# mathwrx/Decouple-and-Couple_Learning_in_Multi-Modal_Brain_Tumor_Segmentation

Measured on AMD Instinct MI355X. Metric: training volumes/sec (4x128^3), higher is better.
Workload: dtype bf16x3 forward (split-bf16 MFMA operands hi.hi+hi.lo+lo.hi: logits within 1e-3 of the fp32 reference) / bf16 data-gradient / bf16 weight-gradient MFMA operands; f32 accumulate, f32 storage, f32 master weights; 1 GPU; configs[1]: 1xMI355X, batch 2 per GPU, 4-modality 128^3 synthetic BraTS patches; fwd + softmax_dice + 4 sub-region/edge losses + bwd + Adam(amsgrad); random-init weights, dropout on; global_batch=2, parallelism=dp1, precision=bf16x3, dgrad_precision=bf16, wgrad_precision=bf16, mode=plan

## Files before the change

### decouple-and-couple_learning_in_multi-modal_brain_tumor_segmentation_amd/csrc/conv_wsp.hip

```cpp
#include "conv_args.h"
#include <cstdlib>
#include <type_traits>

#define WSP_ID 6
#define WSP_IH 6
#define WSP_IW 18
#define WSP_NVOX (WSP_ID * WSP_IH * WSP_IW)
#define WSP_SLOTS 11
#define WSP_NT 2
#define WSP_NBW 14

struct WspWork { int ngroups, slots, tiles, xcd_perm, stat_rows; };

__host__ __device__ constexpr int wsp_tap_bytes(int t) { return (((t / 9) * WSP_IH + (t / 3) % 3) * WSP_IW + t % 3) * 32; }

template <int T>
__global__ __launch_bounds__(512) void convwsp_kernel(const ConvArgsB a, const WspWork wk) {
  constexpr int NT = WSP_NT;
  constexpr int B_IMG = 14 * NT * 1024;
  constexpr int A_IMG = WSP_NVOX * 32;
  constexpr int A_BUF = 2 * A_IMG;
  extern __shared__ float4 lds4[];
  char* lds = reinterpret_cast<char*>(lds4);
  char* const Bh = lds;
// ... 164 lines not shown
      using I0 = std::integral_constant<int, 0>; using I1 = std::integral_constant<int, 1>;
#define WSP_IC(v) std::integral_constant<int, (v)>{}
#define WSP_STEP2(S0)                                                                                          \
      rd_lo(WSP_IC(S0)); rd_hi(WSP_IC((S0) + 1), I1{}); mm(I0{}); __builtin_amdgcn_sched_barrier(0);            \
      rd_lo(WSP_IC((S0) + 1)); if ((S0) + 2 < 14) rd_hi(WSP_IC((S0) + 2 < 14 ? (S0) + 2 : 13), I0{});           \
      mm(I1{}); __builtin_amdgcn_sched_barrier(0);
      rd_hi(I0{}, I0{});
      WSP_STEP2(0) WSP_STEP2(2) WSP_STEP2(4) WSP_STEP2(6) WSP_STEP2(8) WSP_STEP2(10) WSP_STEP2(12)
#undef WSP_STEP2
#undef WSP_IC
    };

    int i = 0;
    for (int t0 = 0; t0 < ntw; t0 += T) {
      const int nk = min(T, ntw - t0);
      for (int c = 0; c < nch; ++c) {
        auto item = [&](auto KK) {
          constexpr int k = decltype(KK)::value;
          if (k == 0 && i > 0) asm volatile("s_barrier" ::: "memory");
          asm volatile("s_barrier" ::: "memory");
          mfma_item(i & 1, KK);
          if (c == nch - 1) epilogue(t_begin + t0 + k, KK);
          ++i;
        };
        item(std::integral_constant<int, 0>{});
        if (T > 1 && nk > 1) item(std::integral_constant<int, (T > 1 ? 1 : 0)>{});
        if (T > 2 && nk > 2) item(std::integral_constant<int, (T > 2 ? 2 : 0)>{});
        if (T > 3 && nk > 3) item(std::integral_constant<int, (T > 3 ? 3 : 0)>{});
      }
    }
    if (a.stats && stats_n >= 0) flush_stats();
  } else {
    const int tg = tid - 256;
    const int ni = ntw * nch;
    struct Item { int tile, chunk; bool first; };
    auto item_of = [&](int it) {
      const int per_round = T * nch;
      const int rd = it / per_round, w = it - rd * per_round;
      const int nk = min(T, ntw - rd * T);
      const int c = w / nk, k = w - c * nk;
      Item o; o.tile = t_begin + rd * T + k; o.chunk = c; o.first = k == 0;
      return o;
    };

    u32x4 wpf[WSP_NBW];
    const uint4* wsrc = a.wpk + (int64_t)g.cls_wbase16[0] * 128;
    auto w_issue = [&](int chunk) {
      int tgo = tg;
      asm volatile("" : "+v"(tgo));
#pragma unroll
      for (int i = 0; i < WSP_NBW; ++i) {
        const int e = tgo + 256 * i;
        const int img = e / (14 * NT * 64), e2 = e - img * (14 * NT * 64);
        const int ln = e2 & 63, blk = e2 >> 6;
        const int j = blk % NT, s = blk / NT;
        const uint4* p = wsrc + ((int64_t)(chunk * 14 + s) * g.ntiles + nt0 + j) * 128 + ln * 2 + img;
        wpf[i] = *reinterpret_cast<const u32x4*>(p);
      }
    };
    auto w_write = [&]() {
      int wb = tg * 16;
      asm volatile("" : "+v"(wb));
#pragma unroll
      for (int i = 0; i < WSP_NBW; ++i) *reinterpret_cast<u32x4*>(Bh + wb + i * 4096) = wpf[i];
    };

    const int q = tg & 3;
    const int vox0 = tg >> 2;
    const int iw_0 = vox0 % WSP_IW, row_0 = vox0 / WSP_IW;
    const bool plain = a.in_scale == nullptr && a.in_slope == 1.f;
    f32x4 pf[WSP_SLOTS];
    f32x4 pf_sc, pf_sh;
    unsigned pf_inb = 0u;
    auto issue = [&](int it) {
      const Item itm = item_of(it);
      const int tile = itm.tile, chunk = itm.chunk;
      const int n = tile / tiles_per_n;
      int bx = tile - n * tiles_per_n;
      const int tw = bx % g.tiles_w; bx /= g.tiles_w;
      const int th = bx % g.tiles_h, td = bx / g.tiles_h;
      const int id0 = td * 4 - 1, ih0 = th * 4 - 1, iw0 = tw * 16 - 1;
      const char* xb = reinterpret_cast<const char*>(a.x + (int64_t)n * g.Di * g.Hi * g.Wi * g.x_ldc + chunk * 16);
      const unsigned ldc4 = (unsigned)g.x_ldc * 4u;
      unsigned inb = 0u;
      int iw = iw_0, row = row_0;
      asm volatile("" : "+v"(iw), "+v"(row));
#pragma unroll
      for (int i = 0; i < WSP_SLOTS; ++i) {
        const int idd = (row * 43) >> 8, ih = row - idd * WSP_IH;
        const int gd = id0 + idd, gh = ih0 + ih, gw = iw0 + iw;
        const bool ok = (row < WSP_ID * WSP_IH) & ((unsigned)gd < (unsigned)g.Di) & ((unsigned)gh < (unsigned)g.Hi) & ((unsigned)gw < (unsigned)g.Wi);
        iw += 10; row += 3;
        if (iw >= WSP_IW) { iw -= WSP_IW; ++row; }
        const unsigned lin = (unsigned)((gd * g.Hi + gh) * g.Wi + gw) * ldc4 + (unsigned)q * 16u;
        const unsigned boff = ok ? lin : (unsigned)q * 16u;
        pf[i] = *reinterpret_cast<const f32x4*>(xb + boff);
        inb |= ok ? (1u << i) : 0u;
      }
      pf_inb = inb;
      const float* scp = a.in_scale ? a.in_scale + (int64_t)n * g.Cin + chunk * 16 : a.x;
      const float* shp = a.in_scale ? a.in_shift + (int64_t)n * g.Cin + chunk * 16 : a.x;
      pf_sc = *reinterpret_cast<const f32x4*>(reinterpret_cast<const char*>(scp) + q * 16);
      pf_sh = *reinterpret_cast<const f32x4*>(reinterpret_cast<const char*>(shp) + q * 16);
    };
    auto convert = [&](int buf) {
      const float slope = a.in_slope;
      const bool has_norm = a.in_scale != nullptr;
      const f32x4 sc = has_norm ? pf_sc : (f32x4){1.f, 1.f, 1.f, 1.f}, sh = has_norm ? pf_sh : (f32x4){0.f, 0.f, 0.f, 0.f};
      const unsigned inb = pf_inb;
      int vbase = (tg >> 2) * 32 + q * 8;
      asm volatile("" : "+v"(vbase));
      char* ah = A0 + buf * A_BUF + vbase;
#pragma unroll
      for (int i = 0; i < WSP_SLOTS; ++i) {
        if (i == WSP_SLOTS - 1 && vox0 + 64 * i >= WSP_NVOX) continue;
        float v0 = pf[i][0], v1 = pf[i][1], v2 = pf[i][2], v3 = pf[i][3];
        if (!plain) {
          v0 = act01(fmaf(v0, sc[0], sh[0]), slope); v1 = act01(fmaf(v1, sc[1], sh[1]), slope);
          v2 = act01(fmaf(v2, sc[2], sh[2]), slope); v3 = act01(fmaf(v3, sc[3], sh[3]), slope);
        }
        uint2 h, l;
        split_bf16(v0, v1, h.x, l.x); split_bf16(v2, v3, h.y, l.y);
        const bool was = (inb >> i) & 1u;
        h.x = was ? h.x : 0u; h.y = was ? h.y : 0u; l.x = was ? l.x : 0u; l.y = was ? l.y : 0u;
        *reinterpret_cast<uint2*>(ah + i * (64 * 32)) = h;
        *reinterpret_cast<uint2*>(ah + A_IMG + i * (64 * 32)) = l;
      }
    };

    __builtin_amdgcn_s_setprio(1);
    if (ni > 0) {
      issue(0);
      w_issue(0);
      convert(0);
      w_write();
      if (ni > 1) issue(1);
    }
    for (int it = 0; it < ni; ++it) {
      if (it > 0 && item_of(it).first) {
        asm volatile("s_barrier" ::: "memory");
        w_write();
      }
      asm volatile("s_waitcnt lgkmcnt(0)\n\ts_barrier" ::: "memory");
      if (it + 1 < ni) {
        convert((it + 1) & 1);
        const Item nx = item_of(it + 1);
        if (nx.first) w_issue(nx.chunk);
        if (it + 2 < ni) issue(it + 2);
      }
    }
  }
}

namespace {
template <int T>
int launch_wsp(const ConvArgsB& a, const WspWork& wk, int grid, hipStream_t st) {
  const size_t lds = (size_t)2 * 14 * WSP_NT * 1024 + (size_t)2 * 2 * WSP_NVOX * 32;
  CWF_MAX_LDS_ONCE((&convwsp_kernel<T>));
  hipLaunchKernelGGL((convwsp_kernel<T>), dim3(grid), dim3(512), lds, st, a, wk);
  CWF_LAUNCH_CHECK();
  return 0;
}
}

static int g_wsp = 1;
extern "C" int cwf_debug_wsp(int v) { const int old = g_wsp; g_wsp = v; return old; }
static long long g_wsp_launches = 0;
extern "C" long long cwf_debug_wsp_launches() { return g_wsp_launches; }
static const int g_wsp_min_cin = 128, g_wsp_min_units = 128;

int cwf_try_conv_wsp(int op, int x3, int cfg_mt, int cfg_wm, ConvArgsB& a, hipStream_t st, int* rc) {
  const ConvGeom& g = a.g;
  if (!g_wsp || !x3 || cwf_ws_takes_x3()) return 0;
  if (op != CWF_CONV3_S1 || a.groups || a.out_scale || a.nb_x) return 0;
  if (g.Cin < 32 || (g.Cin & 15) || (g.Cout & 31)) return 0;
  if ((g.Do & 3) || (g.Ho & 3) || (g.Wo & 15)) return 0;
  if (g.x_ldc < g.Cin || (g.x_ldc & 3)) return 0;
  if ((int64_t)g.Di * g.Hi * g.Wi * g.x_ldc * 4 >= (1ll << 31)) return 0;
  if (a.stats && !(cfg_mt == 1 || (cfg_mt == 4 && cfg_wm == 4))) return 0;
  WspWork wk;
  wk.stat_rows = cfg_mt;
  wk.ngroups = g.Cout / 32;
  if (wk.ngroups > 32) return 0;
  const int64_t tiles = (int64_t)g.N * (g.Do / 4) * (g.Ho / 4) * (g.Wo / 16);
  if (g_wsp == 1 && (g.Cin < g_wsp_min_cin || tiles * wk.ngroups < g_wsp_min_units)) return 0;
  int e = cwf_build_geom(a.g, op, g.N, g.Di, g.Hi, g.Wi, g.Cin, g.x_ldc, g.Do, g.Ho, g.Wo, g.Cout, g.y_ldc, 16);
  if (e) { *rc = e; return 1; }
  wk.tiles = (int)tiles;
  const int per = (32 / wk.ngroups) * wk.ngroups;
  wk.slots = 8 * (per / wk.ngroups);
  wk.xcd_perm = 1;
  if (wk.slots > wk.tiles) { wk.slots = wk.tiles; wk.xcd_perm = 0; }
  const int grid = wk.slots * wk.ngroups;
  const int per_wg = (wk.tiles + wk.slots - 1) / wk.slots;
  *rc = per_wg > 2 ? launch_wsp<4>(a, wk, grid, st) : launch_wsp<2>(a, wk, grid, st);
  if (*rc == 0) ++g_wsp_launches;
  return 1;
}
```

### decouple-and-couple_learning_in_multi-modal_brain_tumor_segmentation_amd/cwf/_lib.py

```python
from __future__ import annotations

import ctypes as C
import os

_HERE = os.path.dirname(os.path.abspath(__file__))
LIB_PATH = os.path.join(_HERE, "libcwf_hip.so")

P = C.c_void_p
I = C.c_int
L = C.c_int64
F = C.c_float
U = C.c_uint32
U64 = C.c_uint64
D = C.c_double

SIGNATURES = {
    "cwf_version": [],
    "cwf_conv": [P, P],
    "cwf_conv_x16_ok": [I, I, I, I, I, I, I],
    "cwf_debug_wsd": [I],
    "cwf_debug_wsd_launches": [],
    "cwf_wgrad": [P, P, P],
    "cwf_gather_split_bf16": [P, I, L, P],
    "cwf_wgrad_nsplit": [I, I, I, I, I, I, I],
    "cwf_wgrad_partial_floats": [I, I, I, I, I, I, I],
    "cwf_wgrad_slab_floats": [I, I, I],
    "cwf_wgrad_reduce": [P, I, L, P, P, P, P],
    "cwf_gather_batched": [P, I, L, P],
    "cwf_in_finalize": [P, P, P, I, L, F, P],
    "cwf_in_stats": [P, I, P, I, L, I, P],
    "cwf_norm_act_add": [P, I, P, P, F, P, I, P, I, I, L, I, P],
    "cwf_in_bwd_stats": [P, I, P, I, P, P, F, P, I, L, I, P],
    "cwf_in_bwd_apply": [P, I, P, I, P, P, F, P, P, I, P, I, I, L, I, P],
    "cwf_in_bwd_apply_ex": [P, I, P, I, P, P, F, P, P, I, P, I, P, P, I, L, I, P],
    "cwf_norm_act_add_ex": [P, I, P, P, F, P, I, P, I, P, I, L, I, P],
    "cwf_to_bf16": [P, I, P, P, F, P, I, L, I, P],
    "cwf_gemm": [P, L, L, L, L, P, L, L, L, L, P, L, L, L, P, P, L, L, L, I, I, I, I, I, F, I, I, P],
    "cwf_layernorm_fwd": [P, P, P, P, P, P, I, I, F, P],
    "cwf_layernorm_bwd": [P, P, P, P, P, P, P, P, I, I, I, P],
    "cwf_softmax_rows": [P, L, I, I, P],
    "cwf_softmax_rows_bwd": [P, P, L, I, I, P],
    "cwf_gelu_bwd": [P, P, P, L, P],
    "cwf_colsum": [P, L, I, I, P, I, P],
    "cwf_window_to_tokens": [P, I, P, I, I, I, I, I, I, I, I, P],
    "cwf_tokens_to_window": [P, P, I, I, I, I, I, I, I, I, I, I, P],
    "cwf_token_scores": [P, P, L, P, I, I, I, P],
    "cwf_topk": [P, P, I, I, I, P],
    "cwf_gather_tokens": [P, P, P, L, P, F, P, I, I, I, I, P],
    "cwf_gather_tokens_bwd": [P, P, P, P, P, L, I, I, I, I, P],
    "cwf_scatter_rows": [P, P, P, L, L, P, L, P, I, I, I, I, P],
    "cwf_scatter_rows_bwd": [P, P, P, P, L, P, I, P, L, L, P, L, I, I, I, I, P],
    "cwf_upsample_softmax": [P, I, P, I, I, I, I, I, I, P],
    "cwf_upsample_softmax_bwd": [P, P, P, I, I, I, I, I, I, I, P, P],
    "cwf_channel_softmax": [P, I, P, L, I, P],
    "cwf_channel_softmax_bwd": [P, P, P, I, L, I, P],
    "cwf_dice_ce_sums": [P, P, U, P, I, L, I, P],
    "cwf_dice_ce_finalize": [P, P, P, I, L, I, P],
    "cwf_dice_ce_bwd": [P, P, U, P, P, P, I, L, I, P],
    "cwf_adam_amsgrad": [P, I, L, C.c_double, C.c_double, C.c_double, C.c_double, C.c_double, I, I, P, P],
    "cwf_adam_amsgrad_scaled": [P, I, L, C.c_double, C.c_double, C.c_double, C.c_double, C.c_double, I, I, P, F, P],
    "cwf_grad_add": [P, P, P, L, P],
    "cwf_grad_norm_clip": [P, L, F, F, P, P, P],
    "cwf_adam_amsgrad_ex": [P, I, L, C.c_double, C.c_double, C.c_double, C.c_double, C.c_double, I, I, P, F, P, P, F, P],
    "cwf_optim_step": [I, P, I, L, C.c_double, C.c_double, P, C.c_double, C.c_double, C.c_double, I, I, P, C.c_double, C.c_double, I, I,
                       F, P, P, F, P],
    "cwf_wgrad_reduce_batched": [P, I, P],
    "cwf_dropout_mask": [P, L, F, F, C.c_uint64, C.c_uint64, P],
    "cwf_mul": [P, P, P, L, P],
    "cwf_add": [P, P, P, L, P],
    "cwf_channel_scale": [P, I, P, P, I, I, L, I, P],
    "cwf_copy_strided": [P, I, P, I, L, I, P],
    "cwf_add3": [P, P, P, P, L, P],
    "cwf_bcast3": [P, P, L, P],
    "cwf_stats_channel_sum": [P, P, I, I, P],
    "cwf_gemm_ex": [P, P],
    "cwf_attn_fwd": [P, L, P, L, I, I, I, I, F, P, U64, F, P],
    "cwf_attn_bwd": [P, L, P, L, P, I, I, I, I, F, P, U64, F, P],
    "cwf_ln_pair_fwd": [P, P, I, P, P, P, P, P, P, P, I, I, F, P],
    "cwf_ln_pair_bwd": [P, P, P, P, P, I, P, P, P, P, P, P, P, P, P, I, I, I, P],
    "cwf_gelu_bwd_drop": [P, P, P, L, P, U64, F, P],
    "cwf_token_scores2": [P, P, L, P, L, P, P, I, I, I, P],
    "cwf_topk_inv": [P, P, P, P, P, P, I, I, I, P],
    "cwf_index_inv": [P, P, I, I, I, P],
    "cwf_gather_multi": [P, I, I, I, I, F, P, F, P],
    "cwf_scatter_inv": [P, P, P, L, L, P, L, P, P, I, I, I, P],
    "cwf_scatter_bwd": [P, P, P, P, P, P, L, L, P, L, P, L, P, L, L, P, L, I, I, I, I, P],
    "cwf_token_grad": [P, P, P, L, P, P, P, L, P, L, P, U64, U64, F, P, I, I, I, I, P],
    "cwf_head_grad": [P, P, P, P, L, P, P, I, I, P],
    "cwf_dice_ce_finalize_multi": [P, P, P, P, I, I, L, I, P],
    "cwf_head_loss_sums": [P, I, I, P, P, P, I, I, I, I, I, P],
    "cwf_head_loss_bwd": [P, I, I, P, P, P, P, P, I, P, I, I, I, I, I, P],
    "cwf_head_loss_bwd_ex": [P, I, I, P, P, P, P, P, I, I, P, I, I, I, I, I, P],
    "cwf_ln_pair_fwd_g": [P, P, I, P, I, P, P, P, I, I, F, P],
    "cwf_ln_pair_bwd_g": [P, P, P, P, P, I, P, I, P, P, P, I, I, I, P],
    "cwf_token_scores2_g": [P, P, P, I, I, P, P, I, I, I, P],
    "cwf_head_grad_g": [P, P, P, P, L, P, P, I, I, I, P],
    "cwf_window_to_tokens_g": [P, I, P, I, I, I, I, I, I, I, I, I, P],
    "cwf_tokens_to_window_g": [P, P, I, I, I, I, I, I, I, I, I, I, P],
    "cwf_cat3_channels": [P, P, P, P, L, I, P],
    "cwf_stitch_windows": [P, P, I, P],
    "cwf_argmax_dice": [P, L, L, L, P, P, P, I, L, P],
    "cwf_argmax_metrics": [P, L, L, L, P, P, P, I, L, P],
    "cwf_region_bits": [P, P, L, P],
    "cwf_hausdorff_workspace": [I, I, I, I, I],
    "cwf_hausdorff": [P, P, I, I, I, I, I, D, D, D, I, I, P, P, P, P, L, P],
    "cwf_surface_metrics_workspace": [I, I, I, I, I],
    "cwf_surface_metrics": [P, P, I, I, I, I, I, D, D, D, I, I, P, I, P, P, P, P, P, P, P, P, L, P],
    "cwf_signed_distance_workspace": [I, I, I, I, I],
    "cwf_signed_distance": [P, P, P, I, I, I, I, I, P, P],
    "cwf_boundary_sums": [P, P, P, P, I, I, L, I, P],
    "cwf_boundary_finalize": [P, P, P, P, I, I, L, P],
    "cwf_boundary_bwd": [P, P, P, P, P, I, I, L, I, P],
    "cwf_topk_ce_workspace": [I, L],
    "cwf_topk_ce": [P, P, U, L, P, P, P, I, L, I, P, P],
    "cwf_topk_ce_bwd": [P, P, U, P, P, P, I, L, I, P],
    "cwf_focal_workspace": [I, L, I],
    "cwf_focal_loss": [P, P, P, I, P, P, P, P, I, L, I, P, P],
    "cwf_focal_loss_bwd": [P, P, P, I, P, P, P, P, I, L, I, P],
    "cwf_lovasz_workspace": [I, L, I],
    "cwf_lovasz": [P, P, P, I, I, P, P, P, P, I, L, P, P],
    "cwf_lovasz_bwd": [P, P, I, P, P, P, I, L, P],
    "cwf_components_workspace": [I, I, I, I, I],
    "cwf_components": [P, I, I, I, I, I, I, P, P, P, P, P, L, P],
    "cwf_postprocess_labels": [P, P, P, P, P, I, I, I, I, I, I, I, I, I, I, I, I, P, P, P],
    "cwf_label_metrics": [P, P, P, L, P],
    "cwf_dilate_bits": [P, P, I, I, I, I, I, I, P, L, P],
    "cwf_lesionwise_workspace": [I, I, I, I, I],
    "cwf_lesionwise": [P, P, I, I, I, I, I, I, L, D, P, P, P, P, P, P, L, P],
    "cwf_lesionwise_ex_workspace": [I, I, I, I, I],
    "cwf_lesionwise_ex": [P, P, I, I, I, I, I, I, L, D, P, I, P, P, P, P, P, P, P, P, L, P],
    "cwf_prepare_batch": [P, I, I, I, I, P, L, P, L, P, L, P],
    "cwf_prepare_batch_affine": [P, I, I, I, I, P, L, P, L, P, L, P],
    "cwf_prepare_batch_elastic": [P, I, I, I, I, P, L, P, L, P, L, P],
    "cwf_augment_intensity": [P, I, I, I, I, P, L, P, L, P, L, P],
    "cwf_augment_acquisition": [P, I, I, I, I, P, L, P, L, P, L, P],
    "cwf_window_gather": [P, P, P, I, I, P],
    "cwf_window_blend": [P, P, P, P, I, I, I, P],
    "cwf_window_finalize": [P, P, P, P, P],
    "cwf_window_gather_box": [P, P, P, P, I, I, P],
    "cwf_window_finalize_box": [P, P, P, P, P, P],
    "cwf_normalize_nonzero": [P, L, P, P],
    "cwf_class_locations_workspace": [L, I],
    "cwf_class_locations": [P, L, P, I, I, P, P, P, P],
    "cwf_nonzero_box_workspace": [I, I, I, I],
    "cwf_nonzero_box": [P, L, I, I, I, I, P, P, P, P],
    "cwf_rng_advance": [P, P],
    "cwf_dropout_mask_rng": [P, L, F, F, P, U64, P],
    "cwf_plan_create": [P, P],
    "cwf_plan_info": [P, P],
    "cwf_plan_run": [P, P, P, I, P, P],
    "cwf_plan_destroy": [P],
    "cwf_plan_marker": [I, P],
    "cwf_plan_schedule": [I, P, P, I, P, P, P, P, P, P, P],
    "cwf_plan_counts": [P, P],
    "cwf_plan_describe": [P, P, P, P, P, P, P, P, P, P],
    "cwf_plan_kernel_name": [P, I, P, I],
}

PLAN_KERNEL, PLAN_MEMSET, PLAN_EMPTY, PLAN_MARKER = 0, 1, 3, 4
PLAN_CLASS_MAIN, PLAN_CLASS_SIDE, PLAN_CLASS_CONVERSION = 0, 1, 2


def plan_describe(lib, plan):
    cnt = (I * 3)()
    check(lib.cwf_plan_counts(plan, cnt), "cwf_plan_counts")
    n, nw, ne = cnt[0], cnt[1], cnt[2]
    kind, stream, marker, record, creation = ((I * n)() for _ in range(5))
    off, wait = (I * (n + 1))(), (I * max(nw, 1))()
    ef, et = (I * max(ne, 1))(), (I * max(ne, 1))()
    check(lib.cwf_plan_describe(plan, kind, stream, marker, record, creation, off, wait, ef, et), "cwf_plan_describe")
    names = []
    for i in range(n):
        ln = lib.cwf_plan_kernel_name(plan, i, None, 0)
        if ln < 0:
# ... 152 lines not shown
```

### include/cwf_hip.h

```cpp
#ifndef CWF_HIP_H
#define CWF_HIP_H
#include <stdint.h>
#ifdef __cplusplus
extern "C" {
#endif

#define CWF_E_BADARG   (-1)
#define CWF_E_TOOLARGE (-2)
#define CWF_E_ALIGN    (-3)

int cwf_version(void);
const char* cwf_arch(void);

enum { CWF_CONV3_S1 = 0, CWF_CONV3_S2 = 1, CWF_CONV1 = 2, CWF_CONVT2 = 3, CWF_CONV3_S2_DGRAD = 4, CWF_CONVT2_DGRAD = 5 };
enum { CWF_FP32 = 0, CWF_BF16X3 = 1, CWF_BF16 = 2 };

struct cwf_conv_args {
  int op, precision;
  const float* x; int x_ldc; const void* wpk; const float* bias; float* y; int y_ldc;
  const float* in_scale; const float* in_shift; float in_slope;
  const float* residual; int r_ldc; const float* out_scale; double* stats;
  const float* nb_x; int nb_ldc; const float* nb_scale; const float* nb_shift; float nb_slope;
  const void* x16; const void* zero16; void* y16;
  const float* w_raw;
  int groups, x_goff, y_goff; const void* wpk_g[3]; const float* bias_g[3];
  int N, Di, Hi, Wi, Cin, Do, Ho, Wo, Cout;
};
int cwf_conv(const struct cwf_conv_args* args , void* stream);
int cwf_conv_x16_ok(int op, int N, int D, int H, int W, int Cin, int Cout);
int cwf_debug_wsd(int v);
long long cwf_debug_wsd_launches(void);

int cwf_wgrad_nsplit(int op, int N, int Do, int Ho, int Wo, int Cin, int Cout);
int64_t cwf_wgrad_partial_floats(int op, int N, int Do, int Ho, int Wo, int Cin, int Cout);
int64_t cwf_wgrad_slab_floats(int op, int Cin, int Cout);
struct cwf_wgrad_args {
  int op, precision;
  const float* x; int x_ldc; const float* in_scale; const float* in_shift; float in_slope;
  const float* dy; int dy_ldc;
  const float* dy_scale; const void* xa16; const void* dy16; const void* zero16;
  float* partial;
  int groups; const float* x_g[3]; const float* dy_g[3]; float* partial_g[3];
  int N, Di, Hi, Wi, Cin, Do, Ho, Wo, Cout;
};
int cwf_wgrad(const struct cwf_wgrad_args* args , int* nsplit_used , void* stream);
int cwf_wgrad_reduce(const float* partial, int nsplit, int64_t slab_floats,
                     const int32_t* inv_map, float* dW, float* db, void* stream);
struct cwf_wgrad_reduce_desc { const float* partial; const int32_t* inv; float* dW; float* db; int64_t slab; int32_t nsplit; int32_t pad_; };
int cwf_wgrad_reduce_batched(const struct cwf_wgrad_reduce_desc* table, int nlayers, void* stream);

struct cwf_gather_desc { const float* src; float* dst; const int32_t* map; int64_t n; };

int cwf_gather_split_bf16(const struct cwf_gather_desc* table, int nlayers, int64_t max_n, void* stream);

int cwf_gather_batched(const struct cwf_gather_desc* table, int nlayers, int64_t max_n, void* stream);

int cwf_in_finalize(const double* stats, float* scale, float* shift, int NC, int64_t V, float eps, void* stream);
int cwf_in_stats(const float* x, int x_ldc, double* stats, int N, int64_t V, int C, void* stream);
int cwf_norm_act_add(const float* x, int x_ldc, const float* scale, const float* shift, float slope,
                     const float* residual, int r_ldc, float* y, int y_ldc, int N, int64_t V, int C, void* stream);
int cwf_in_bwd_stats(const float* dy, int dy_ldc, const float* x, int x_ldc, const float* scale, const float* shift,
                     float slope, double* sums, int N, int64_t V, int C, void* stream);
int cwf_in_bwd_apply(const float* dy, int dy_ldc, const float* x, int x_ldc, const float* scale, const float* shift,
                     float slope, const double* sums, const float* dx_add, int a_ldc, float* dx, int dx_ldc,
                     int N, int64_t V, int C, void* stream);

int cwf_in_bwd_apply_ex(const float* dy, int dy_ldc, const float* x, int x_ldc, const float* scale, const float* shift,
                        float slope, const double* sums, const float* dx_add, int a_ldc, float* dx, int dx_ldc,
                        void* dx16, void* xa16, int N, int64_t V, int C, void* stream);
int cwf_norm_act_add_ex(const float* x, int x_ldc, const float* scale, const float* shift, float slope,
                        const float* residual, int r_ldc, float* y, int y_ldc, void* y16, int N, int64_t V, int C, void* stream);
int cwf_to_bf16(const float* x, int x_ldc, const float* scale, const float* shift, float slope, void* y16,
                int N, int64_t V, int C, void* stream);
int cwf_gemm(const float* A, int64_t sa_m, int64_t sa_k, int64_t sa_zb, int64_t sa_zh,
             const float* B, int64_t sb_k, int64_t sb_n, int64_t sb_zb, int64_t sb_zh,
             float* C, int64_t sc_m, int64_t sc_zb, int64_t sc_zh,
             const float* bias, const float* residual, int64_t sr_m, int64_t sr_zb, int64_t sr_zh,
             int M, int Nn, int K, int ZB, int ZH, float alpha, int act, int accumulate, void* stream);
struct cwf_gemm_args {
  const float* A; int64_t sa_m, sa_k, sa_zb, sa_zh;
  const float* B; int64_t sb_k, sb_n, sb_zb, sb_zh;
  float* C; int64_t sc_m, sc_zb, sc_zh;
  const float* bias; const float* residual; int64_t sr_m, sr_zb, sr_zh;
  int M, N, K, ZB, ZH; float alpha; int act; int accumulate;
  const float* A2; int split_n;
  const float* B2; int split_m;
  float* C2;
  float* rowsum; int rowsum_acc;
  const uint64_t* rng;
  uint64_t a_drop_off, a_drop_n; float a_drop_p, a_drop_p2;
  uint64_t c_drop_off, c_drop_n; float c_drop_p, c_drop_p2;
  const float* B_tab[4]; const float* bias_tab[4]; float* C_tab[4]; float* rowsum_tab[4];
};
int cwf_gemm_ex(const struct cwf_gemm_args* args , void* stream);

int cwf_attn_fwd(const float* qkv, int64_t ld, float* o, int64_t ldo, int Z, int T, int E, int heads, float scale,
                 const uint64_t* rng, uint64_t drop_off, float drop_p, void* stream);
int cwf_attn_bwd(const float* qkv, int64_t ld, const float* d_o, int64_t ldo, float* dqkv, int Z, int T, int E, int heads,
                 float scale, const uint64_t* rng, uint64_t drop_off, float drop_p, void* stream);

int cwf_ln_pair_fwd(const float* x, const float* x2, int perm_T, const float* g1, const float* b1, const float* g2, const float* b2,
                    float* ya, float* yb, float* stats, int rows, int E, float eps, void* stream);
struct cwf_ln_group_params { const float* g1[4]; const float* b1[4]; const float* g2[4]; const float* b2[4];
                             float* dg1[4]; float* db1[4]; float* dg2[4]; float* db2[4]; };
int cwf_ln_pair_fwd_g(const float* x, const float* x2, int perm_T, const struct cwf_ln_group_params* h_params, int groups,
                      float* ya, float* yb, float* stats, int rows, int E, float eps, void* stream);
int cwf_ln_pair_bwd_g(const float* dy, const float* da, const float* db, const float* x, const float* x2, int perm_T,
                      const struct cwf_ln_group_params* h_params, int groups, const float* stats, float* dx, float* dx2,
                      int rows, int E, int accumulate_params, void* stream);
int cwf_ln_pair_bwd(const float* dy, const float* da, const float* db, const float* x, const float* x2, int perm_T,
                    const float* g1, const float* g2, const float* stats, float* dx, float* dx2,
                    float* dg1, float* db1, float* dg2, float* db2, int rows, int E, int accumulate_params, void* stream);
int cwf_gelu_bwd_drop(const float* z, const float* dh, float* dz, int64_t n, const uint64_t* rng, uint64_t off, float p, void* stream);

int cwf_layernorm_fwd(const float* x, const float* gamma, const float* beta, float* y, float* mean, float* rstd,
                      int rows, int E, float eps, void* stream);
int cwf_layernorm_bwd(const float* dy, const float* x, const float* gamma, const float* mean, const float* rstd,
                      float* dx, float* dgamma, float* dbeta, int rows, int E, int accumulate, void* stream);
int cwf_softmax_rows(float* s, int64_t rows, int cols, int ld, void* stream);
int cwf_softmax_rows_bwd(const float* p, float* dp_inout, int64_t rows, int cols, int ld, void* stream);
int cwf_gelu_bwd(const float* x, const float* dy, float* dx, int64_t n, void* stream);
int cwf_colsum(const float* x, int64_t rows, int cols, int ld, float* out, int accumulate, void* stream);

int cwf_window_to_tokens(const float* x, int x_ldc, float* tok, int B, int D, int H, int W, int C,
                         int p0, int p1, int p2, void* stream);
int cwf_tokens_to_window(const float* tok, float* x, int x_ldc, int B, int D, int H, int W, int C,
                         int p0, int p1, int p2, int accumulate, void* stream);
int cwf_token_scores(const float* feats, const float* query, int64_t query_bstride, float* score,
                     int B, int T, int E, void* stream);
int cwf_topk(const float* score, int32_t* index, int B, int T, int k, void* stream);
int cwf_gather_tokens(const float* feats, const int32_t* index, const float* head, int64_t head_bstride,
                      const float* keep, float pe_odd, float* seq, int B, int T, int k, int E, void* stream);
int cwf_gather_tokens_bwd(const float* dseq, const int32_t* index, const float* keep, float* dfeats, float* dhead,
                          int64_t dhead_bstride, int B, int T, int k, int E, void* stream);
int cwf_scatter_rows(const float* feats, const int32_t* index, const float* rows, int64_t rows_ld, int64_t rows_bs,
                     const float* gate, int64_t gate_bs, float* out, int B, int T, int k, int E, void* stream);
int cwf_scatter_rows_bwd(const float* dout, const int32_t* index, const float* scat, const float* gate, int64_t gate_bs,
                         float* dfeats, int accumulate, float* drows, int64_t drows_ld, int64_t drows_bs,
                         float* dgate, int64_t dgate_bs, int B, int T, int k, int E, void* stream);

int cwf_token_scores2(const float* feats, const float* q1, int64_t q1_bstride, const float* q2, int64_t q2_bstride,
                      float* s1, float* s2, int B, int T, int E, void* stream);
int cwf_token_scores2_g(const float* feats, const float* const* h_q1, const float* const* h_q2, int groups, int group_B,
                        float* s1, float* s2, int B, int T, int E, void* stream);
int cwf_topk_inv(const float* score0, int32_t* index0, int32_t* inv0, const float* score1, int32_t* index1, int32_t* inv1,
                 int B, int T, int k, void* stream);
int cwf_index_inv(const int32_t* index, int32_t* inv, int B, int T, int k, void* stream);
struct cwf_gather_job { const float* feats; const int32_t* index; const float* head; float* out;
                        int64_t head_bstride, out_bstride; int T; uint64_t drop_off;
                        const float* head_g[4]; int group_B;  };
int cwf_gather_multi(const struct cwf_gather_job* jobs , int njobs, int B, int k, int E, float pe_odd,
                     const uint64_t* rng, float p, void* stream);
int cwf_scatter_inv(const float* feats, const int32_t* inv, const float* rows, int64_t rows_ld, int64_t rows_bs,
                    const float* gate, int64_t gate_bs, float* gated, float* scat, int B, int T, int E, void* stream);
int cwf_scatter_bwd(const float* dgated, const float* dscat, const float* feats, const int32_t* inv, const int32_t* index,
                    const float* rows, int64_t rows_ld, int64_t rows_bs, const float* gate, int64_t gate_bs,
                    const float* dgate_extra, int64_t extra_bs, float* drows, int64_t drows_ld, int64_t drows_bs,
                    float* dgate, int64_t dgate_bs, int B, int T, int k, int E, void* stream);
int cwf_token_grad(const float* dgated, const float* dscat, const float* gate, int64_t gate_bs,
                   const int32_t* inv_p, const int32_t* inv_q, const float* dseq_p, int64_t dseq_p_bs,
                   const float* dseq_q, int64_t dseq_q_bs, const uint64_t* rng, uint64_t drop_off_p, uint64_t drop_off_q, float p,
                   float* dfeats, int B, int T, int k, int E, void* stream);
int cwf_head_grad(const float* a1, const float* c1, const float* a2, const float* c2, int64_t bstride,
                  float* out1, float* out2, int B, int E, void* stream);
int cwf_head_grad_g(const float* a1, const float* c1, const float* a2, const float* c2, int64_t bstride,
                    float* const* h_out1, float* const* h_out2, int groups, int group_B, int E, void* stream);
int cwf_window_to_tokens_g(const float* x, int x_ldc, float* tok, int groups, int B, int D, int H, int W, int C,
                           int p0, int p1, int p2, void* stream);
int cwf_tokens_to_window_g(const float* tok, float* x, int x_ldc, int groups, int B, int D, int H, int W, int C,
                           int p0, int p1, int p2, void* stream);
int cwf_cat3_channels(const float* x0, const float* x1, const float* x2, float* y, int64_t nvox, int C, void* stream);

int cwf_upsample_softmax(const float* logit, int l_ldc, float* prob, int N, int D, int H, int W, int C, int scale,
                         void* stream);
int cwf_upsample_softmax_bwd(const float* dprob, const float* prob, float* dlogit, int dl_ldc,
                             int N, int D, int H, int W, int C, int scale, float* workspace, void* stream);
int cwf_channel_softmax(const float* logit, int l_ldc, float* prob, int64_t nvox, int C, void* stream);
int cwf_channel_softmax_bwd(const float* dprob, const float* prob, float* dlogit, int dl_ldc, int64_t nvox, int C,
                            void* stream);

int cwf_dice_ce_sums(const float* prob, const int64_t* label, uint32_t posmask, double* sums,
                     int N, int64_t V, int C, void* stream);
int cwf_dice_ce_finalize(const double* sums, float* loss, float* coef, int N, int64_t V, int C, void* stream);
int cwf_dice_ce_finalize_multi(const double* sums, float* loss, float* coef, float* total, int nmaps, int N, int64_t V, int C, void* stream);
// ... 225 lines not shown
```

Before: 118.8 volumes/s.

## Add per-unit warp-specialized conv kernel for small-tile 3x3x3 layers

Adds a variant of the warp-specialized bf16x3 conv kernel that assigns one (tile, 16-channel group) unit per workgroup. It double-buffers activations and weights, with 4 producer waves staging data and 4 MFMA waves computing. A planner selects it when the tile count, Cout and unit count are small (deep, low-resolution layers). The aim is more workgroups and better occupancy on those layers than the slot-based persistent kernel gives, at the cost of reloading the halo for each channel group and more launch-level scheduling.

```diff
diff --git a/decouple-and-couple_learning_in_multi-modal_brain_tumor_segmentation_amd/csrc/conv_wsp.hip b/decouple-and-couple_learning_in_multi-modal_brain_tumor_segmentation_amd/csrc/conv_wsp.hip
--- a/decouple-and-couple_learning_in_multi-modal_brain_tumor_segmentation_amd/csrc/conv_wsp.hip
+++ b/decouple-and-couple_learning_in_multi-modal_brain_tumor_segmentation_amd/csrc/conv_wsp.hip
@@ -340,6 +340,249 @@
   }
 }
 
+#define WSU_A_IMG (WSP_NVOX * 32)
+#define WSU_B_IMG (14 * 1024)
+#define WSU_BUF (2 * WSU_A_IMG + 2 * WSU_B_IMG)
+#define WSU_LDS (2 * WSU_BUF + 4 * 16 * 2 * (int)sizeof(double))
+struct WspUnitWork { int ngroups, stat_rows; };
+
+__global__ __launch_bounds__(512) void convwsp_unit_kernel(const ConvArgsB a, const WspUnitWork wk) {
+  constexpr int A_IMG = WSU_A_IMG, B_IMG = WSU_B_IMG, BUF = WSU_BUF;
+  extern __shared__ float4 lds4[];
+  char* lds = reinterpret_cast<char*>(lds4);
+  const ConvGeom& g = a.g;
+  const int nch = g.nchunks;
+  const int tid = threadIdx.x, lane = tid & 63;
+  const int wave = __builtin_amdgcn_readfirstlane(tid >> 6);
+
+  int b = blockIdx.x;
+  if ((gridDim.x & 7) == 0) b = (b & 7) * (gridDim.x >> 3) + (b >> 3);
+  const int nt0 = b % wk.ngroups, tile = b / wk.ngroups;
+  const int tiles_per_n = g.tiles_d * g.tiles_h * g.tiles_w;
+  const int n = tile / tiles_per_n;
+  int bx = tile - n * tiles_per_n;
+  const int tw = bx % g.tiles_w; bx /= g.tiles_w;
+  const int th = bx % g.tiles_h, td = bx / g.tiles_h;
+
+  if (wave < 4) {
+    const int wl = wave;
+    const int r = lane & 15, kq = lane >> 4;
+    const bool second = (kq >> 1) != 0;
+    const int a_lane = ((wl * WSP_IH) * WSP_IW + r) * 32 + (kq & 1) * 16;
+    const int b_lane = 2 * A_IMG + lane * 16;
+
+    f32x4 acc[4];
+#pragma unroll
+    for (int m = 0; m < 4; ++m) acc[m] = (f32x4){0.f, 0.f, 0.f, 0.f};
+
+    auto mfma_item = [&](int buf) {
+      const char* ah0 = lds + buf * BUF + a_lane;
+      const char* al0 = ah0 + A_IMG;
+      const char* bh = lds + buf * BUF + b_lane;
+      const char* bl = bh + B_IMG;
+      uint4 fa[2][4], fb[2], fl[4], fbl;
+      auto rd_hi = [&](auto S, auto P) {
+        constexpr int s = decltype(S)::value, p = decltype(P)::value;
+        constexpr int c0 = wsp_tap_bytes(2 * s), c1 = wsp_tap_bytes(2 * s + 1 < 27 ? 2 * s + 1 : 2 * s);
+        const int to = second ? c1 : c0;
+#pragma unroll
+        for (int m = 0; m < 4; ++m) fa[p][m] = *reinterpret_cast<const uint4*>(ah0 + to + m * (WSP_IW * 32));
+        fb[p] = *reinterpret_cast<const uint4*>(bh + s * 1024);
+      };
+      auto rd_lo = [&](auto S) {
+        constexpr int s = decltype(S)::value;
+        constexpr int c0 = wsp_tap_bytes(2 * s), c1 = wsp_tap_bytes(2 * s + 1 < 27 ? 2 * s + 1 : 2 * s);
+        const int to = second ? c1 : c0;
+#pragma unroll
+        for (int m = 0; m < 4; ++m) fl[m] = *reinterpret_cast<const uint4*>(al0 + to + m * (WSP_IW * 32));
+        fbl = *reinterpret_cast<const uint4*>(bl + s * 1024);
+      };
+      auto mm = [&](auto P) {
+        constexpr int p = decltype(P)::value;
+#pragma unroll
+        for (int m = 0; m < 4; ++m)
+          acc[m] = __builtin_amdgcn_mfma_f32_16x16x32_bf16(__builtin_bit_cast(bf16x8, fa[p][m]), __builtin_bit_cast(bf16x8, fb[p]), acc[m], 0, 0, 0);
+#pragma unroll
+        for (int m = 0; m < 4; ++m)
+          acc[m] = __builtin_amdgcn_mfma_f32_16x16x32_bf16(__builtin_bit_cast(bf16x8, fa[p][m]), __builtin_bit_cast(bf16x8, fbl), acc[m], 0, 0, 0);
+#pragma unroll
+        for (int m = 0; m < 4; ++m)
+          acc[m] = __builtin_amdgcn_mfma_f32_16x16x32_bf16(__builtin_bit_cast(bf16x8, fl[m]), __builtin_bit_cast(bf16x8, fb[p]), acc[m], 0, 0, 0);
+      };
+      using I0 = std::integral_constant<int, 0>; using I1 = std::integral_constant<int, 1>;
+#define WSU_IC(v) std::integral_constant<int, (v)>{}
+#define WSU_STEP2(S0)                                                                                          \
+      rd_lo(WSU_IC(S0)); rd_hi(WSU_IC((S0) + 1), I1{}); mm(I0{}); __builtin_amdgcn_sched_barrier(0);            \
+      rd_lo(WSU_IC((S0) + 1)); if ((S0) + 2 < 14) rd_hi(WSU_IC((S0) + 2 < 14 ? (S0) + 2 : 13), I0{});           \
+      mm(I1{}); __builtin_amdgcn_sched_barrier(0);
+      rd_hi(I0{}, I0{});
+      WSU_STEP2(0) WSU_STEP2(2) WSU_STEP2(4) WSU_STEP2(6) WSU_STEP2(8) WSU_STEP2(10) WSU_STEP2(12)
+#undef WSU_STEP2
+#undef WSU_IC
+    };
+
+    for (int i = 0; i < nch; ++i) {
+      asm volatile("s_barrier" ::: "memory");
+      mfma_item(i & 1);
+    }
+
+    float s1 = 0.f, s2 = 0.f;
+    double d1 = 0.0, d2 = 0.0;
+    auto fold_stats = [&]() {
+      float u1 = s1, u2 = s2;
+      u1 += __shfl_xor(u1, 16, 64); u1 += __shfl_xor(u1, 32, 64);
+      u2 += __shfl_xor(u2, 16, 64); u2 += __shfl_xor(u2, 32, 64);
+      d1 += (double)u1; d2 += (double)u2;
+      s1 = 0.f; s2 = 0.f;
+    };
+    const float bv = a.bias ? a.bias[nt0 * 16 + r] : 0.f;
+    auto epi = [&](auto HR, auto HT) {
+      constexpr bool HAS_RES = decltype(HR)::value, HAS_STATS = decltype(HT)::value;
+      unsigned yo[4], ro[4];
+#pragma unroll
+      for (int i = 0; i < 4; ++i) {
+        yo[i] = (unsigned)((kq * 4 + i) * g.y_ldc + nt0 * 16 + r) * 4u; asm volatile("" : "+v"(yo[i]));
+        if (HAS_RES) { ro[i] = (unsigned)((kq * 4 + i) * a.r_ldc + nt0 * 16 + r) * 4u; asm volatile("" : "+v"(ro[i])); }
+      }
+      const int od = td * 4 + wl;
+      float rv[4][4];
+      if (HAS_RES) {
+#pragma unroll
+        for (int m = 0; m < 4; ++m) {
+          const int64_t vox0 = (((int64_t)n * g.Do + od) * g.Ho + th * 4 + m) * g.Wo + tw * 16;
+          const char* rb = reinterpret_cast<const char*>(a.residual + vox0 * a.r_ldc);
+#pragma unroll
+          for (int i = 0; i < 4; ++i) rv[m][i] = *reinterpret_cast<const float*>(rb + ro[i]);
+        }
+      }
+#pragma unroll
+      for (int m = 0; m < 4; ++m) {
+        const int64_t vox0 = (((int64_t)n * g.Do + od) * g.Ho + th * 4 + m) * g.Wo + tw * 16;
+        char* yb = reinterpret_cast<char*>(a.y + vox0 * g.y_ldc);
+#pragma unroll
+        for (int i = 0; i < 4; ++i) {
+          float v = acc[m][i] + bv;
+          if (HAS_RES) v += rv[m][i];
+          *reinterpret_cast<float*>(yb + yo[i]) = v;
+          if (HAS_STATS) { s1 += v; s2 = fmaf(v, v, s2); }
+        }
+        if (HAS_STATS && (wk.stat_rows == 1 || m == 3)) fold_stats();
+      }
+    };
+    using T_ = std::true_type; using F_ = std::false_type;
+    if (a.residual) { if (a.stats) epi(T_{}, T_{}); else epi(T_{}, F_{}); }
+    else            { if (a.stats) epi(F_{}, T_{}); else epi(F_{}, F_{}); }
+    if (a.stats) {
+      double* red = reinterpret_cast<double*>(lds + 2 * BUF);
+      if (kq == 0) {
+        red[(wl * 16 + r) * 2 + 0] = d1;
+        red[(wl * 16 + r) * 2 + 1] = d2;
+      }
+      asm volatile("s_waitcnt lgkmcnt(0)\n\ts_barrier" ::: "memory");
+      if (tid < 32) {
+        const int which = tid & 1, cr = tid >> 1;
+        double sum = 0.0;
+#pragma unroll
+        for (int w = 0; w < 4; ++w) sum += red[(w * 16 + cr) * 2 + which];
+        atomic_add_f64(a.stats + ((int64_t)n * g.Cout + nt0 * 16 + cr) * 2 + which, sum);
+      }
+    }
+  } else {
+    constexpr int TG = 256, DV = TG / 4;
+    constexpr int SLOTS = WSP_SLOTS;
+    constexpr int NBW = 2 * B_IMG / 16 / TG;
+    static_assert(SLOTS * DV >= WSP_NVOX && NBW * TG * 16 == 2 * B_IMG, "staging covers the halo and the weight chunk exactly");
+    const int tg = tid - 256;
+    const uint4* wsrc = a.wpk + (int64_t)g.cls_wbase16[0] * 128;
+    const int q = tg & 3;
+    const int vox0 = tg >> 2;
+    const int id0 = td * 4 - 1, ih0 = th * 4 - 1, iw0 = tw * 16 - 1;
+    unsigned xoff[SLOTS], woff[NBW];
+    unsigned pf_inb = 0u;
+    {
+      const unsigned ldc4 = (unsigned)g.x_ldc * 4u;
+      int iw = vox0 % WSP_IW, row = vox0 / WSP_IW;
+#pragma unroll
+      for (int i = 0; i < SLOTS; ++i) {
+        const int idd = (row * 43) >> 8, ih = row - idd * WSP_IH;
+        const int gd = id0 + idd, gh = ih0 + ih, gw = iw0 + iw;
+        const bool ok = (row < WSP_ID * WSP_IH) & ((unsigned)gd < (unsigned)g.Di) & ((unsigned)gh < (unsigned)g.Hi) & ((unsigned)gw < (unsigned)g.Wi);
+        iw += DV % WSP_IW; row += DV / WSP_IW;
+        if (iw >= WSP_IW) { iw -= WSP_IW; ++row; }
+        const unsigned lin = (unsigned)((gd * g.Hi + gh) * g.Wi + gw) * ldc4 + (unsigned)q * 16u;
+        xoff[i] = ok ? lin : (unsigned)q * 16u;
+        pf_inb |= ok ? (1u << i) : 0u;
+      }
+#pragma unroll
+      for (int i = 0; i < NBW; ++i) {
+        const int e = tg + TG * i;
+        const int img = e >= B_IMG / 16 ? 1 : 0, e2 = e - img * (B_IMG / 16);
+        const int ln = e2 & 63, s = e2 >> 6;
+        woff[i] = (unsigned)((s * g.ntiles + nt0) * 128 + ln * 2 + img) * 16u;
+      }
+    }
+    const bool plain = a.in_scale == nullptr && a.in_slope == 1.f;
+    const bool has_norm = a.in_scale != nullptr;
+    f32x4 pf[SLOTS];
+    u32x4 wpf[NBW];
+    f32x4 pf_sc, pf_sh;
+    const char* xsample = reinterpret_cast<const char*>(a.x + (int64_t)n * g.Di * g.Hi * g.Wi * g.x_ldc);
+    const char* scs = reinterpret_cast<const char*>(has_norm ? a.in_scale + (int64_t)n * g.Cin : a.x);
+    const char* shs = reinterpret_cast<const char*>(has_norm ? a.in_shift + (int64_t)n * g.Cin : a.x);
+    const int pstep = has_norm ? 64 : 0;
+    auto issue = [&](int chunk) {
+      const char* wb = reinterpret_cast<const char*>(wsrc + (int64_t)chunk * 14 * g.ntiles * 128);
+      const char* xb = xsample + chunk * 64;
+#pragma unroll
+      for (int i = 0; i < NBW; ++i) wpf[i] = *reinterpret_cast<const u32x4*>(wb + woff[i]);
+#pragma unroll
+      for (int i = 0; i < SLOTS; ++i) pf[i] = *reinterpret_cast<const f32x4*>(xb + xoff[i]);
+      pf_sc = *reinterpret_cast<const f32x4*>(scs + chunk * pstep + q * 16);
+      pf_sh = *reinterpret_cast<const f32x4*>(shs + chunk * pstep + q * 16);
+    };
+    auto convert = [&](int buf) {
+      const float slope = a.in_slope;
+      const f32x4 sc = has_norm ? pf_sc : (f32x4){1.f, 1.f, 1.f, 1.f}, sh = has_norm ? pf_sh : (f32x4){0.f, 0.f, 0.f, 0.f};
+      const unsigned inb = pf_inb;
+      int vbase = buf * BUF + (tg >> 2) * 32 + q * 8;
+      asm volatile("" : "+v"(vbase));
+      char* ah = lds + vbase;
+#pragma unroll
+      for (int i = 0; i < SLOTS; ++i) {
+        if (DV * (i + 1) > WSP_NVOX && vox0 + DV * i >= WSP_NVOX) continue;
+        float v0 = pf[i][0], v1 = pf[i][1], v2 = pf[i][2], v3 = pf[i][3];
+        if (!plain) {
+          v0 = act01(fmaf(v0, sc[0], sh[0]), slope); v1 = act01(fmaf(v1, sc[1], sh[1]), slope);
+          v2 = act01(fmaf(v2, sc[2], sh[2]), slope); v3 = act01(fmaf(v3, sc[3], sh[3]), slope);
+        }
+        uint2 h, l;
+        split_bf16(v0, v1, h.x, l.x); split_bf16(v2, v3, h.y, l.y);
+        const bool was = (inb >> i) & 1u;
+        h.x = was ? h.x : 0u; h.y = was ? h.y : 0u; l.x = was ? l.x : 0u; l.y = was ? l.y : 0u;
+        *reinterpret_cast<uint2*>(ah + i * (DV * 32)) = h;
+        *reinterpret_cast<uint2*>(ah + A_IMG + i * (DV * 32)) = l;
+      }
+      int wb = buf * BUF + 2 * A_IMG + tg * 16;
+      asm volatile("" : "+v"(wb));
+#pragma unroll
+      for (int i = 0; i < NBW; ++i) *reinterpret_cast<u32x4*>(lds + wb + i * (TG * 16)) = wpf[i];
+    };
+
+    __builtin_amdgcn_s_setprio(1);
+    issue(0);
+    convert(0);
+    if (nch > 1) issue(1);
+    for (int it = 0; it < nch; ++it) {
+      asm volatile("s_waitcnt lgkmcnt(0)\n\ts_barrier" ::: "memory");
+      if (it + 1 < nch) {
+        convert((it + 1) & 1);
+        if (it + 2 < nch) issue(it + 2);
+      }
+    }
+    if (a.stats) asm volatile("s_barrier" ::: "memory");
+  }
+}
+
 namespace {
 template <int T>
 int launch_wsp(const ConvArgsB& a, const WspWork& wk, int grid, hipStream_t st) {
@@ -349,6 +592,12 @@
   CWF_LAUNCH_CHECK();
   return 0;
 }
+int launch_wsp_unit(const ConvArgsB& a, const WspUnitWork& wk, int grid, hipStream_t st) {
+  CWF_MAX_LDS_ONCE((&convwsp_unit_kernel));
+  hipLaunchKernelGGL(convwsp_unit_kernel, dim3(grid), dim3(512), (size_t)WSU_LDS, st, a, wk);
+  CWF_LAUNCH_CHECK();
+  return 0;
+}
 }
 
 static int g_wsp = 1;
@@ -356,6 +605,49 @@
 static long long g_wsp_launches = 0;
 extern "C" long long cwf_debug_wsp_launches() { return g_wsp_launches; }
 static const int g_wsp_min_cin = 128, g_wsp_min_units = 128;
+static int g_wsp_unit = 1;
+extern "C" int cwf_debug_wsp_unit(int v) { const int old = g_wsp_unit; g_wsp_unit = v; return old; }
+static const int g_wsp_unit_max_tiles = 64, g_wsp_unit_max_cout = 128, g_wsp_unit_max_units = 256;
+
+namespace {
+struct WspPlan { int taken, unit, nt, grid, lds, tmpl; WspWork wk; };
+WspPlan wsp_plan(int N, int D, int H, int W, int Cin, int Cout) {
+  WspPlan p = {};
+  if (!g_wsp || cwf_ws_takes_x3()) return p;
+  if (N < 1 || D < 1 || H < 1 || W < 1) return p;
+  if (Cin < 32 || (Cin & 15) || Cout < 32 || (Cout & 31)) return p;
+  if ((D & 3) || (H & 3) || (W & 15)) return p;
+  p.wk.ngroups = Cout / 32;
+  if (p.wk.ngroups > 32) return p;
+  const int64_t tiles = (int64_t)N * (D / 4) * (H / 4) * (W / 16);
+  if (g_wsp == 1 && (Cin < g_wsp_min_cin || tiles * p.wk.ngroups < g_wsp_min_units)) return p;
+  p.taken = 1;
+  p.wk.tiles = (int)tiles;
+  const int64_t units = tiles * (Cout / 16);
+  if ((g_wsp_unit == 2 && units <= (1 << 24)) ||
+      (g_wsp_unit == 1 && tiles <= g_wsp_unit_max_tiles && Cout <= g_wsp_unit_max_cout && units <= g_wsp_unit_max_units)) {
+    p.unit = 1; p.nt = 1;
+    p.grid = (int)units;
+    p.lds = WSU_LDS;
+    return p;
+  }
+  const int per = (32 / p.wk.ngroups) * p.wk.ngroups;
+  p.wk.slots = 8 * (per / p.wk.ngroups);
+  p.wk.xcd_perm = 1;
+  if (p.wk.slots > p.wk.tiles) { p.wk.slots = p.wk.tiles; p.wk.xcd_perm = 0; }
+  p.nt = WSP_NT;
+  p.grid = p.wk.slots * p.wk.ngroups;
+  p.lds = 2 * 14 * WSP_NT * 1024 + 2 * 2 * WSP_NVOX * 32;
+  p.tmpl = (p.wk.tiles + p.wk.slots - 1) / p.wk.slots > 2 ? 4 : 2;
+  return p;
+}
+}
+extern "C" int cwf_debug_wsp_plan(int N, int D, int H, int W, int Cin, int Cout, int* out5) {
+  if (!out5) return 1;
+  const WspPlan p = wsp_plan(N, D, H, W, Cin, Cout);
+  out5[0] = p.taken; out5[1] = p.unit; out5[2] = p.nt; out5[3] = p.grid; out5[4] = p.lds;
+  return 0;
+}
 
 int cwf_try_conv_wsp(int op, int x3, int cfg_mt, int cfg_wm, ConvArgsB& a, hipStream_t st, int* rc) {
   const ConvGeom& g = a.g;
@@ -366,22 +658,19 @@
   if (g.x_ldc < g.Cin || (g.x_ldc & 3)) return 0;
   if ((int64_t)g.Di * g.Hi * g.Wi * g.x_ldc * 4 >= (1ll << 31)) return 0;
   if (a.stats && !(cfg_mt == 1 || (cfg_mt == 4 && cfg_wm == 4))) return 0;
-  WspWork wk;
-  wk.stat_rows = cfg_mt;
-  wk.ngroups = g.Cout / 32;
-  if (wk.ngroups > 32) return 0;
-  const int64_t tiles = (int64_t)g.N * (g.Do / 4) * (g.Ho / 4) * (g.Wo / 16);
-  if (g_wsp == 1 && (g.Cin < g_wsp_min_cin || tiles * wk.ngroups < g_wsp_min_units)) return 0;
+  WspPlan p = wsp_plan(g.N, g.Do, g.Ho, g.Wo, g.Cin, g.Cout);
+  if (!p.taken) return 0;
   int e = cwf_build_geom(a.g, op, g.N, g.Di, g.Hi, g.Wi, g.Cin, g.x_ldc, g.Do, g.Ho, g.Wo, g.Cout, g.y_ldc, 16);
   if (e) { *rc = e; return 1; }
-  wk.tiles = (int)tiles;
-  const int per = (32 / wk.ngroups) * wk.ngroups;
-  wk.slots = 8 * (per / wk.ngroups);
-  wk.xcd_perm = 1;
-  if (wk.slots > wk.tiles) { wk.slots = wk.tiles; wk.xcd_perm = 0; }
-  const int grid = wk.slots * wk.ngroups;
-  const int per_wg = (wk.tiles + wk.slots - 1) / wk.slots;
-  *rc = per_wg > 2 ? launch_wsp<4>(a, wk, grid, st) : launch_wsp<2>(a, wk, grid, st);
+  if (p.unit) {
+    WspUnitWork uw;
+    uw.ngroups = g.Cout / 16;
+    uw.stat_rows = cfg_mt;
+    *rc = launch_wsp_unit(a, uw, p.grid, st);
+  } else {
+    p.wk.stat_rows = cfg_mt;
+    *rc = p.tmpl == 4 ? launch_wsp<4>(a, p.wk, p.grid, st) : launch_wsp<2>(a, p.wk, p.grid, st);
+  }
   if (*rc == 0) ++g_wsp_launches;
   return 1;
 }
diff --git a/decouple-and-couple_learning_in_multi-modal_brain_tumor_segmentation_amd/cwf/_lib.py b/decouple-and-couple_learning_in_multi-modal_brain_tumor_segmentation_amd/cwf/_lib.py
--- a/decouple-and-couple_learning_in_multi-modal_brain_tumor_segmentation_amd/cwf/_lib.py
+++ b/decouple-and-couple_learning_in_multi-modal_brain_tumor_segmentation_amd/cwf/_lib.py
@@ -20,6 +20,8 @@
     "cwf_conv_x16_ok": [I, I, I, I, I, I, I],
     "cwf_debug_wsd": [I],
     "cwf_debug_wsd_launches": [],
+    "cwf_debug_wsp_unit": [I],
+    "cwf_debug_wsp_plan": [I, I, I, I, I, I, P],
     "cwf_wgrad": [P, P, P],
     "cwf_gather_split_bf16": [P, I, L, P],
     "cwf_wgrad_nsplit": [I, I, I, I, I, I, I],
diff --git a/include/cwf_hip.h b/include/cwf_hip.h
--- a/include/cwf_hip.h
+++ b/include/cwf_hip.h
@@ -30,6 +30,8 @@
 int cwf_conv_x16_ok(int op, int N, int D, int H, int W, int Cin, int Cout);
 int cwf_debug_wsd(int v);
 long long cwf_debug_wsd_launches(void);
+int cwf_debug_wsp_unit(int v);
+int cwf_debug_wsp_plan(int N, int D, int H, int W, int Cin, int Cout, int* out5);
 
 int cwf_wgrad_nsplit(int op, int N, int Do, int Ho, int Wo, int Cin, int Cout);
 int64_t cwf_wgrad_partial_floats(int op, int N, int Do, int Ho, int Wo, int Cin, int Cout);
```

Result: no change. 119.7 volumes/s, median of 6 (+0.7%).
